# theartful/polychase

Measured on AMD Instinct MI355X. Metric: optical-flow frames/sec, higher is better.
Workload: dtype u8/int32 fixed-point + f32 2x2 solve; 1 GPU; C2 1920x1080 300-frame synthetic clip, 3-level pyramidal LK (max_level=3); width=1920, height=1080, max_level=3, window=10, pairs_per_frame=8, frames_per_gpu=1877, arith=opencv_x86, parallelism=single GPU

## Files before the change

### polychase_amd/csrc/hip/api.hip

```cpp
#include "api_internal.hpp"

#include <dirent.h>
#include <unistd.h>

#include <cstring>
#include <mutex>

namespace pc {
std::string& last_error() {
    thread_local std::string e;
    return e;
}
}

namespace pc_api {

int collect_timing(pc_context* c) {
    if (c->ranges.empty()) return PC_OK;
    PC_HIP(c->sync_side_streams());
    PC_HIP(hipStreamSynchronize(c->stream));
    std::vector<std::pair<float, float>> spans[PC_K_COUNT];
    hipEvent_t const origin = c->ranges.front().a;
    for (auto& r : c->ranges) {
        float ms = 0.f, t0 = 0.f;
// ... 105 lines not shown

static bool tiled_response(const pc_gftt_options& opt) {
    static const bool force_general = getenv("POLYCHASE_GFTT_GENERAL") && atoi(getenv("POLYCHASE_GFTT_GENERAL")) == 1;
    return opt.block_size == 3 && opt.gradient_size == 3 && !opt.use_harris && !force_general;
}

static bool fused_detection(const pc_gftt_options& opt) {
    return tiled_response(opt) && opt.min_distance >= 1 && !(opt.min_distance > pc::kSuppressMaxTableRadius);
}

static int corner_response(pc_context* ctx, const pc_frame* f, DetectScratch& d, const pc::GfttGrid& grid, const pc_gftt_options& opt,
                           uint32_t* cell_max) {
    const int fma = ((ctx->arith & PC_ARITH_SOBEL_FMA) ? 1 : 0) | ((ctx->arith & PC_ARITH_SOBEL_ROW_FMA) ? 2 : 0);
    if (tiled_response(opt)) {
        pc::launch_min_eig(f->levels[0], d.eig.p, grid, cell_max, fma, ctx->work);
        return PC_OK;
    }
    PC_HIP(d.cov.ensure((size_t)3 * f->w * f->h));
    const bool two_pass = opt.block_size >= pc::kBoxRowsFromBlock;
    if (two_pass) PC_HIP(d.box_rows.ensure((size_t)3 * f->w * f->h));
    if (!pc::launch_corner_response(f->levels[0], d.eig.p, d.cov.p, two_pass ? d.box_rows.p : nullptr, grid, cell_max, opt.block_size, opt.gradient_size, opt.use_harris != 0, opt.harris_k,
                                    fma, ctx->work))
        return fail(PC_E_INVALID, "gradient_size must be 3, 5, 7 (Sobel) or -1 (Scharr)");
    return PC_OK;
}

int detect_reserve(pc_context* ctx, int w, int h, DetectScratch& d, const pc_gftt_options* opt) {
    const size_t npx = (size_t)w * h;
    const size_t cand_cap = std::min(npx, npx / 4 + 65536);
    PC_HIP(d.eig.ensure(npx));
    PC_HIP(d.cstate.ensure(npx + 16));
    PC_HIP(d.keys.ensure(cand_cap));
    PC_HIP(d.keys_bucketed.ensure(cand_cap));
    if (opt && fused_detection(*opt)) PC_HIP(d.key_slots.ensure((size_t)pc::kSortBuckets * pc::kBucketSlots, true));
    PC_HIP(d.keys_sorted.ensure(cand_cap));
    d.cand_cap = (uint32_t)std::min<size_t>(d.keys.cap, std::min(d.keys_bucketed.cap, d.keys_sorted.cap));
    d.ticket_stride = ticket_stride(w, h, d.cand_cap);
    d.counter_words = kTicketsAt + 3 * (int)d.ticket_stride;
    PC_HIP(d.counters.ensure((size_t)d.counter_words));
    PC_HIP(d.bucket_offsets.ensure(pc::kSortBuckets + 1));
    PC_HIP(d.per_block.ensure((size_t)pc::suppress_num_blocks(d.cand_cap) + 1));
    PC_HIP(d.h_counters.ensure(kHostCells));
    if (!d.ev_b) PC_HIP(hipEventCreateWithFlags(&d.ev_b, hipEventDisableTiming));
    (void)ctx;
    return PC_OK;
}

static int upload_suppression_offsets(pc_context* ctx, const pc_gftt_options& opt) {
    if (!(opt.min_distance >= 1) || ctx->sup_min_distance == opt.min_distance) return PC_OK;
    if (opt.min_distance > pc::kSuppressMaxTableRadius) return PC_OK;
    const std::vector<int2> offs = suppression_offsets(opt.min_distance);
    PC_HIP(ctx->sup_offsets.ensure(offs.size() + 1));
    PC_HIP(hipStreamSynchronize(ctx->work));
    PC_HIP(hipMemcpy(ctx->sup_offsets.p, offs.data(), offs.size() * sizeof(int2), hipMemcpyHostToDevice));
    ctx->n_sup_offsets = (int)offs.size();
    int R = 0;
    for (const int2& o : offs) R = std::max(R, std::max(std::abs(o.x), std::abs(o.y)));
    std::vector<int> hw((size_t)2 * R + 1, -1);
    for (const int2& o : offs) hw[(size_t)(o.y + R)] = std::max(hw[(size_t)(o.y + R)], std::abs(o.x));
    hw[(size_t)R] = std::max(hw[(size_t)R], 0);
    size_t covered = 0;
    for (int v : hw) covered += v >= 0 ? (size_t)(2 * v + 1) : 0;
    if (covered != offs.size() + 1) return fail(PC_E_INVALID, "suppression neighbourhood is not row-contiguous");
    PC_HIP(ctx->sup_rows.ensure(hw.size()));
    PC_HIP(hipMemcpy(ctx->sup_rows.p, hw.data(), hw.size() * sizeof(int), hipMemcpyHostToDevice));
    ctx->sup_R = R;
    ctx->sup_min_distance = opt.min_distance;
    return PC_OK;
}

static int ensure_perm_capacity(pc_frame* f, int n) {
    if (f->perm_cap >= n) return PC_OK;
    if (f->d_perm) PC_HIP(hipFree(f->d_perm));
    f->d_perm = nullptr;
    f->perm_cap = 0;
    const int want = std::max(n + n / 2, 1024);
    PC_HIP(hipMalloc(&f->d_perm, (size_t)want * 2 * sizeof(uint32_t)));
    f->perm_cap = want;
    return PC_OK;
}

int detect_enqueue(pc_context* ctx, pc_frame* f, const pc::GfttGrid& grid, const pc_gftt_options& opt, DetectScratch& d,
                   DevBuf<uint32_t>& hist, bool full_launch) {
    const int w = f->w, h = f->h;
    int rc = detect_reserve(ctx, w, h, d, &opt);
    if (rc != PC_OK) return rc;
    if ((rc = upload_suppression_offsets(ctx, opt)) != PC_OK) return rc;
    if (f->kp_cap < 4096 && (rc = ensure_kp_capacity(f, 4096)) != PC_OK) return rc;
    if ((rc = ensure_perm_capacity(f, f->kp_cap)) != PC_OK) return rc;
    PC_HIP(hist.ensure((size_t)pc::bin_num_tiles(w, h) + 1));
    uint32_t* const cnt = d.counters.p;
    if (!d.cleared) PC_HIP(hipMemsetAsync(cnt, 0, (size_t)d.counter_words * sizeof(uint32_t), ctx->work));
    uint32_t* const tickets = cnt + kTicketsAt;
    d.cleared = false;
    const uint32_t n_launch = (ctx->cand_hint > 0 && !full_launch) ? std::min(ctx->cand_hint, d.cand_cap) : d.cand_cap;
    const bool large_radius = opt.min_distance > pc::kSuppressMaxTableRadius;
    const bool fused = fused_detection(opt);
    {
        ScopedTimer t(ctx, PC_K_MINEIG);
        if ((rc = corner_response(ctx, f, d, grid, opt, cnt + kCellMaxAt)) != PC_OK) return rc;
    }
    {
        ScopedTimer t(ctx, PC_K_NMS);
        pc::launch_nms(d.eig.p, w, h, grid, cnt + kCellMaxAt, opt.quality_level, d.keys.p, d.cand_cap, cnt + kCntCand, d.cstate.p,
                       cnt + kCntSortParams, cnt + kHistAt, tickets, d.bucket_offsets.p, hist.p, ctx->work,
                       fused ? d.key_slots.p : nullptr, fused ? d.per_block.p : nullptr, pc::suppress_num_blocks(n_launch));
    }
    {
        ScopedTimer t(ctx, PC_K_SORT);
        if (fused)
            pc::launch_bucket_sort_slots(d.key_slots.p, d.bucket_offsets.p, d.keys_sorted.p, cnt + kCntOverflow, ctx->work);
        else
            pc::launch_bucket_sort(d.keys.p, d.cand_cap, n_launch, cnt + kCntCand, cnt + kCntSortParams, d.bucket_offsets.p,
                                   cnt + kCursorAt, d.keys_bucketed.p, d.keys_sorted.p, cnt + kCntOverflow, ctx->work);
    }
    const uint32_t limit = opt.max_corners > 0 ? std::min<uint32_t>((uint32_t)opt.max_corners, (uint32_t)f->kp_cap) : (uint32_t)f->kp_cap;
    if (large_radius) PC_HIP(d.sup_grid.ensure((size_t)pc::suppress_large_grid_words(w, h, opt.min_distance)));
    if (fused) {
        ScopedTimer t(ctx, PC_K_SUPPRESS);
        pc::launch_suppress_compact(d.keys_sorted.p, n_launch, cnt + kCntCand, w, h, d.eig.p, d.cstate.p, ctx->sup_offsets.p,
                                    ctx->n_sup_offsets, ctx->sup_rows.p, ctx->sup_R, d.per_block.p, cnt + kCntStuck, limit, f->d_kps,
                                    cnt + kCntKps, hist.p, cnt + kCntOverflow, tickets + d.ticket_stride, ctx->work);
    } else {
        ScopedTimer t(ctx, PC_K_SUPPRESS);
        pc::launch_suppress_and_compact(d.keys_sorted.p, n_launch, cnt + kCntCand, w, h, d.eig.p, d.cstate.p, ctx->sup_offsets.p,
                                        ctx->n_sup_offsets, ctx->sup_rows.p, ctx->sup_R, opt.min_distance >= 1, d.per_block.p,
                                        cnt + kCntStuck, limit, f->d_kps,
                                        cnt + kCntKps, hist.p, cnt + kCntOverflow, tickets + d.ticket_stride, d.ticket_stride,
                                        opt.min_distance, large_radius ? d.sup_grid.p : nullptr, ctx->work);
    }
    pc::launch_spatial_bins_counted(f->d_kps, (int)std::min<uint32_t>(limit, n_launch), cnt + kCntKps, w, h, hist.p, f->d_perm,
                                    f->d_perm + f->perm_cap, cnt, d.h_counters.p, kHostCells, ctx->work);
    PC_HIP(hipEventRecord(d.ev_b, ctx->work));
    f->n_kps = -1;
    f->n_cands = -1;
    f->perm_valid = false;
    return PC_OK;
}

static int detect_slow_path(pc_context* ctx, pc_frame* f, const pc::GfttGrid& grid, const pc_gftt_options& opt, DetectScratch& d,
                            DevBuf<uint32_t>& hist) {
    const int w = f->w, h = f->h;
    const uint32_t npx = (uint32_t)((size_t)w * h);
    PC_HIP(hipStreamSynchronize(ctx->work));
    PC_HIP(d.keys.ensure(npx));
    PC_HIP(d.keys_sorted.ensure(npx));
    PC_HIP(d.per_block.ensure((size_t)pc::suppress_num_blocks(npx) + 1));
    PC_HIP(hist.ensure((size_t)pc::bin_num_tiles(w, h) + 1));
    uint32_t* const cnt = d.counters.p;
    d.cleared = false;
    PC_HIP(hipMemsetAsync(cnt, 0, (size_t)d.counter_words * sizeof(uint32_t), ctx->work));
    uint32_t* const tickets = cnt + kTicketsAt;
    if (int crc = corner_response(ctx, f, d, grid, opt, cnt + kCellMaxAt)) return crc;
// ... 831 lines not shown
```

### polychase_amd/csrc/hip/kernels.hpp

```cpp
#pragma once

#include "bvh.hpp"
#include "common.hpp"

namespace pc {

int helper_prio_arg();
void set_helper_prio(int hi);

void launch_rgb2gray(const uint8_t* rgb, size_t rgb_pitch, const Level& l0, hipStream_t s);
void launch_rgbf32_to_gray(const float* rgb, size_t rgb_pitch, int channels, const Level& l0, hipStream_t s);
void launch_copy_gray(const uint8_t* gray, size_t gray_pitch, const Level& l0, hipStream_t s);
void launch_pyrdown(const Level& src, const Level& dst, hipStream_t s);
void launch_border(const Level& l, int win, hipStream_t s);
void launch_widen(const Level& l, int win, hipStream_t s);
void launch_scharr(const Level& l, hipStream_t s);

enum LevelSourceKind { SRC_PYR = 0, SRC_RGB8 = 1, SRC_GRAY8 = 2, SRC_RGBF32 = 3 };
struct LevelSource {
    int kind;
    const uint8_t* src;
    size_t src_pitch;
    int channels;
    int aligned;
    Level parent;
    uint32_t* clear;
    int clear_words;
};
void launch_level(const LevelSource& in, const Level& out, int win, hipStream_t s);

struct GfttGrid {
    int rows, cols;
    int cell_w, cell_h;
};
constexpr int kMaxGridCells = 1024;
void launch_min_eig(const Level& l0, float* eig, const GfttGrid& g, uint32_t* cell_max, int sobel_fma, hipStream_t s);
constexpr int kBoxRowsFromBlock = 12;
bool launch_corner_response(const Level& l0, float* eig, float* cov, double* box_rows, const GfttGrid& g, uint32_t* cell_max, int block_size, int gradient_size,
                            bool harris, double harris_k, int sobel_fma, hipStream_t s);
constexpr int kSortBuckets = 8192;
constexpr int kBucketSlots = 512;
void launch_nms(const float* eig, int w, int h, const GfttGrid& g, const uint32_t* cell_max, double quality_level,
                unsigned long long* keys, uint32_t cap, uint32_t* counter, uint8_t* cstate, uint32_t* sort_params, uint32_t* hist,
                uint32_t* ticket, uint32_t* bucket_offsets, uint32_t* bin_hist, hipStream_t s,
                unsigned long long* slots = nullptr, uint32_t* zero = nullptr, int zero_words = 0);
void launch_bucket_sort(const unsigned long long* keys, uint32_t cap, uint32_t n_launch, const uint32_t* counter, const uint32_t* sort_params,
                        const uint32_t* offsets, uint32_t* cursor, unsigned long long* scratch, unsigned long long* out,
                        uint32_t* overflow, hipStream_t s);
void launch_bucket_sort_slots(const unsigned long long* slots, const uint32_t* offsets, unsigned long long* out, uint32_t* overflow,
                              hipStream_t s);
int suppress_num_blocks(uint32_t n);
void launch_suppress_and_compact(const unsigned long long* keys, uint32_t n_max, const uint32_t* n_dev, int w, int h, const float* eig,
                                 uint8_t* cstate, const int2* offsets, int n_offsets, const int* row_hw, int R, bool suppress,
                                 uint32_t* per_block,
                                 uint32_t* stuck, uint32_t max_corners, float2* xy, uint32_t* n_out, uint32_t* bin_hist,
                                 uint32_t* overflow, uint32_t* tickets, uint32_t ticket_stride, double large_min_distance, uint32_t* large_grid,
                                 hipStream_t s);
void launch_suppress_compact(const unsigned long long* keys, uint32_t n_max, const uint32_t* n_dev, int w, int h, const float* eig,
                             uint8_t* cstate, const int2* offsets, int n_offsets, const int* row_hw, int R, uint32_t* lookback,
                             uint32_t* stuck, uint32_t max_corners, float2* xy, uint32_t* n_out, uint32_t* bin_hist,
                             uint32_t* overflow, uint32_t* ticket, hipStream_t s);
constexpr double kSuppressMaxTableRadius = 64.0;
int suppress_large_grid_words(int w, int h, double min_distance);
hipError_t sort_keys_desc(void* temp, size_t& temp_bytes, unsigned long long* keys_in,
                          unsigned long long* keys_out, uint32_t n, hipStream_t s);

constexpr int kMaxLevels = 16;
struct LKParams {
    Level src[kMaxLevels];
    const uint8_t* tgt[8][kMaxLevels];
    const uint16_t* tgt16[8][kMaxLevels];
    int n_targets;
    int max_level;
    int n;
    const float2* pts;
    const uint32_t* perm;
    int blocks_per_xcd;
    int max_iters;
    double eps_sq;
    float min_eig_thr;
    float min_eig_num_thr;
    float4* out_rec;
    unsigned long long* prof;
    uint32_t* gate;
    uint32_t gate_value;
    int x86_order;
    unsigned long long* x86_stats;
};
void launch_lk_gate(const uint32_t* gate, uint32_t value, uint32_t* timed_out, hipStream_t s);
__device__ __forceinline__ void lk_signal_dispatched(const LKParams& p) {
    if (p.gate && blockIdx.x == gridDim.x - 1 && threadIdx.x == 0)
        __hip_atomic_store(p.gate, p.gate_value, __ATOMIC_RELAXED, __HIP_MEMORY_SCOPE_AGENT);
// ... 135 lines not shown
```

### polychase_amd/csrc/hip/kernels_gftt.hip

```cpp
#include <algorithm>
#include <cstring>
#include <type_traits>
#include <rocprim/device/device_radix_sort.hpp>

#include <cmath>

#include "kernels.hpp"

namespace pc {

constexpr int TW = 64, TH = 16;
constexpr int GH = TH + 4, G_PITCH = 72;
constexpr int CW = TW + 2, CH = TH + 2;

template <bool ROW_FMA>
__device__ __forceinline__ float smooth_row(float a, float b, float c, float f1, float f0) {
    float t = f1 * a;
    if (ROW_FMA) {
        t = __fmaf_rn(f0, b, t);
        t = __fmaf_rn(f1, c, t);
    } else {
        t += f0 * b;
        t += f1 * c;
    }
// ... 496 lines not shown
    if (box_rows) hipLaunchKernelGGL(box_rows_kernel, grid, dim3(256), 0, s, cov, l0.w, l0.h, block_size, box_rows, helper_prio_arg());
    hipLaunchKernelGGL(box_response_kernel, grid, dim3(256), 0, s, cov, (const double*)box_rows, l0.w, l0.h, block_size, harris ? ((sobel_fma & 1) ? 2 : 1) : 0, harris_k, eig, g, cell_max,
                       helper_prio_arg());
    return true;
}

constexpr int NMS_SUB = 4;

struct SortRange {
    uint32_t hi, shift;
};
__host__ __device__ __forceinline__ SortRange make_sort_range(uint32_t lo, uint32_t hi) {
    SortRange r;
    r.hi = hi;
    r.shift = 0;
    const uint32_t span = hi > lo ? hi - lo : 0u;
    while ((span >> r.shift) >= (uint32_t)kSortBuckets) r.shift++;
    return r;
}
__device__ __forceinline__ uint32_t bucket_of(uint32_t ord, const SortRange& r) {
    const uint32_t d = r.hi > ord ? r.hi - ord : 0u;
    const uint32_t b = d >> r.shift;
    return b < (uint32_t)kSortBuckets ? b : (uint32_t)kSortBuckets - 1u;
}

__global__ __launch_bounds__(256) void nms_kernel(const float* __restrict__ eig, int w, int h, GfttGrid g,
                                                  const uint32_t* __restrict__ cell_max, double quality_level,
                                                  unsigned long long* __restrict__ keys, uint32_t cap,
                                                  uint32_t* __restrict__ counter, uint8_t* __restrict__ cstate,
                                                  uint32_t* __restrict__ sort_params, uint32_t* __restrict__ hist,
                                                  uint32_t* __restrict__ ticket, uint32_t* __restrict__ bucket_offsets,
                                                  uint32_t* __restrict__ bin_hist, int n_tiles,
                                                  unsigned long long* __restrict__ slots, uint32_t* __restrict__ zero, int zero_words,
                                                  int hi_prio) {
    helper_priority(hi_prio);
    __shared__ float s_thr[kMaxGridCells];
    __shared__ uint32_t s_hi, s_lo;
    __shared__ float s_v[CH][CW + 2];
    __shared__ uint32_t s_wave[4];
    __shared__ uint32_t s_base;
    const int tid = threadIdx.x;
    const int x0 = blockIdx.x * TW;
    const int ncells = g.rows * g.cols;
    if (tid == 0) {
        s_hi = 0u;
        s_lo = 0xffffffffu;
    }
    __syncthreads();
    for (int i = tid; i < ncells; i += 256) {
        const float mx = ordered_to_float(cell_max[i]);
        s_thr[i] = (float)((double)mx * quality_level);
        atomicMax(&s_hi, cell_max[i]);
        atomicMin(&s_lo, float_to_ordered(s_thr[i] > 0.f ? s_thr[i] : 0.f));
    }
    __syncthreads();
    const SortRange range = make_sort_range(s_lo, s_hi);
    if (blockIdx.x == 0 && blockIdx.y == 0) {
        if (tid == 0) {
            sort_params[0] = range.hi;
            sort_params[1] = range.shift;
        }
        if (bin_hist)
            for (int i = tid; i < n_tiles; i += 256) bin_hist[i] = 0u;
    }
    for (int i = (blockIdx.y * gridDim.x + blockIdx.x) * 256 + tid; i < zero_words; i += gridDim.x * gridDim.y * 256) zero[i] = 0u;
    const int r = tid >> 4, q = tid & 15;
    const int x = x0 + 4 * q;
// ... 93 lines not shown
        s_base = total ? atomicAdd(counter, total) : 0u;
    }
    __syncthreads();
    if (cnt != 0) {
        uint32_t pos = s_base + incl - cnt;
        for (int wv = 0; wv < wave; wv++) pos += s_wave[wv];
#pragma unroll
        for (int sub = 0; sub < NMS_SUB; sub++) {
            const int y = (blockIdx.y * NMS_SUB + sub) * TH + r;
#pragma unroll
            for (int i = 0; i < 4; i++) {
                if (flags & (1u << (4 * sub + i))) {
                    const uint32_t ord = float_to_ordered(vals[sub][i]);
                    if (pos < cap) {
                        const unsigned long long key = ((unsigned long long)ord << 32) | (unsigned long long)(uint32_t)(y * w + x + i);
                        const uint32_t b = bucket_of(ord, range);
                        if (slots) {
                            const uint32_t at = atomicAdd(&hist[b], 1u);
                            slots[(size_t)b * kBucketSlots + min(at, (uint32_t)kBucketSlots - 1u)] = key;
                        } else {
                            keys[pos] = key;
                            atomicAdd(&hist[b], 1u);
                        }
                    }
                    pos++;
                }
            }
        }
    }
    if (ticket && last_workgroup(ticket, gridDim.x * gridDim.y)) {
        __shared__ uint32_t s_scan[256];
        const uint32_t total = scan_exclusive_256_fixed<kSortBuckets / 256>(hist, bucket_offsets, s_scan);
        if (tid == 0) bucket_offsets[kSortBuckets] = total;
    }
}

void launch_nms(const float* eig, int w, int h, const GfttGrid& g, const uint32_t* cell_max, double quality_level,
                unsigned long long* keys, uint32_t cap, uint32_t* counter, uint8_t* cstate, uint32_t* sort_params, uint32_t* hist,
                uint32_t* ticket, uint32_t* bucket_offsets, uint32_t* bin_hist, hipStream_t s,
                unsigned long long* slots, uint32_t* zero, int zero_words) {
    dim3 grid((w + TW - 1) / TW, (h + NMS_SUB * TH - 1) / (NMS_SUB * TH));
    hipLaunchKernelGGL(nms_kernel, grid, dim3(256), 0, s, eig, w, h, g, cell_max, quality_level, keys, cap, counter, cstate,
                       sort_params, hist, ticket, bucket_offsets, bin_hist, bin_hist ? bin_num_tiles(w, h) : 0, slots, zero,
                       zero ? zero_words : 0, helper_prio_arg());
}

constexpr int kBucketLds = 512;

__global__ __launch_bounds__(256) void bucket_scatter_kernel(const unsigned long long* __restrict__ keys, uint32_t cap,
                                                             const uint32_t* __restrict__ counter, const uint32_t* __restrict__ sort_params,
                                                             const uint32_t* __restrict__ offsets, uint32_t* __restrict__ cursor,
                                                             unsigned long long* __restrict__ out, int hi_prio) {
    helper_priority(hi_prio);
    const uint32_t n = min(*counter, cap);
    SortRange range;
    range.hi = sort_params[0];
    range.shift = sort_params[1];
    for (uint32_t i = blockIdx.x * blockDim.x + threadIdx.x; i < n; i += gridDim.x * blockDim.x) {
        const unsigned long long key = keys[i];
        const uint32_t b = bucket_of((uint32_t)(key >> 32), range);
        out[offsets[b] + atomicAdd(&cursor[b], 1u)] = key;
    }
}

constexpr int kBucketsPerWave = 4;

constexpr int kSortWaves = 4;
static_assert(kBucketSlots == kBucketLds, "a bucket beyond its slots is a bucket beyond the fast path");
template <bool SLOTS>
__global__ __launch_bounds__(64 * kSortWaves) void bucket_sort_kernel(const unsigned long long* __restrict__ in, const uint32_t* __restrict__ offsets,
                                                         unsigned long long* __restrict__ out, uint32_t* __restrict__ overflow, int hi_prio) {
    helper_priority(hi_prio);
    __shared__ unsigned long long s_all[kSortWaves][kBucketLds];
    const int lane = threadIdx.x & 63, wave = threadIdx.x >> 6;
    unsigned long long* const s_keys = s_all[wave];
    const int b0 = (blockIdx.x * kSortWaves + wave) * kBucketsPerWave;
    if (b0 >= kSortBuckets) return;
// ... 73 lines not shown
                        uint32_t* overflow, hipStream_t s) {
    const unsigned blocks = std::max(1u, std::min<unsigned>(1024u, (n_launch + 255u) / 256u));
    hipLaunchKernelGGL(bucket_scatter_kernel, dim3(blocks), dim3(256), 0, s, keys, cap, counter, sort_params, offsets, cursor, scratch, helper_prio_arg());
    hipLaunchKernelGGL(bucket_sort_kernel<false>, dim3((kSortBuckets / kBucketsPerWave + kSortWaves - 1) / kSortWaves), dim3(64 * kSortWaves), 0, s, scratch,
                       offsets, out, overflow, helper_prio_arg());
}
void launch_bucket_sort_slots(const unsigned long long* slots, const uint32_t* offsets, unsigned long long* out, uint32_t* overflow,
                              hipStream_t s) {
    hipLaunchKernelGGL(bucket_sort_kernel<true>, dim3((kSortBuckets / kBucketsPerWave + kSortWaves - 1) / kSortWaves), dim3(64 * kSortWaves), 0, s, slots,
                       offsets, out, overflow, helper_prio_arg());
}

struct AcceptedScan {
    uint32_t* ticket;
    uint32_t* n_out;
    uint32_t* overflow;
    uint32_t max_corners;
};
__device__ __forceinline__ void finish_accepted_scan(uint32_t* per_block, const AcceptedScan& fin, uint32_t n_max, const uint32_t* n_dev) {
    if (!last_workgroup(fin.ticket, gridDim.x)) return;
    __shared__ uint32_t s_scan[256];
    if (threadIdx.x == 0 && n_dev && fin.overflow && *n_dev > n_max) atomicOr(fin.overflow, 4u);
    const uint32_t total = scan_exclusive_256(per_block, per_block, (int)gridDim.x, s_scan);
    if (threadIdx.x == 0) *fin.n_out = (fin.max_corners > 0 && total > fin.max_corners) ? fin.max_corners : total;
}

constexpr uint8_t CS_CAND = 1, CS_ACCEPTED = 2, CS_REJECTED = 3;
constexpr int SUP_NB = 12;
constexpr int SUP_BLOCK = 256;

__device__ __forceinline__ uint8_t cs_load(const uint8_t* p) { return __hip_atomic_load(p, __ATOMIC_RELAXED, __HIP_MEMORY_SCOPE_AGENT); }
__device__ __forceinline__ void cs_store(uint8_t* p, uint8_t v) { __hip_atomic_store(p, v, __ATOMIC_RELAXED, __HIP_MEMORY_SCOPE_AGENT); }

__device__ __forceinline__ bool suppress_decide(const unsigned long long* __restrict__ keys, uint32_t n, int w, int h,
                                                const float* __restrict__ eig, uint8_t* cstate, const int2* __restrict__ offsets,
                                                int n_offsets, const int* __restrict__ row_hw, int R, uint32_t* __restrict__ stuck,
                                                uint32_t* idx_out) {
    const uint32_t i = blockIdx.x * SUP_BLOCK + threadIdx.x;
    const bool live = i < n;
    uint32_t my_val = 0, my_idx = 0;
    uint32_t nb[SUP_NB];
    int n_nb = 0;
    bool overflow = false;
    int x = 0, y = 0;
    if (live) {
        const unsigned long long key = keys[i];
        my_val = (uint32_t)(key >> 32);
        my_idx = (uint32_t)key;
        y = (int)(my_idx / (uint32_t)w);
        x = (int)(my_idx - (uint32_t)y * (uint32_t)w);
        for (int dy = -R; dy <= R; dy++) {
            const int ny = y + dy, hw = row_hw[dy + R];
            if (ny < 0 || ny >= h || hw < 0) continue;
            const uint32_t lin0 = (uint32_t)(ny * w + max(x - hw, 0)), lin1 = (uint32_t)(ny * w + min(x + hw, w - 1));
            for (uint32_t a = lin0 & ~3u; a <= lin1; a += 4u) {
                uint32_t v = *reinterpret_cast<const uint32_t*>(cstate + a);
                if (a < lin0) v &= 0xffffffffu << (8u * (lin0 - a));
                if (a + 3u > lin1) v &= 0xffffffffu >> (8u * (a + 3u - lin1));
                while (v) {
                    const uint32_t b = (uint32_t)(__ffs((int)v) - 1) >> 3;
                    v &= ~(0xffu << (8u * b));
                    const uint32_t nidx = a + b;
                    if (nidx == my_idx) continue;
                    const uint32_t nval = float_to_ordered(eig[nidx]);
                    if (!(nval > my_val || (nval == my_val && nidx > my_idx))) continue;
                    if (n_nb < SUP_NB) {
#pragma unroll
                        for (int k = 0; k < SUP_NB; k++)
                            if (k == n_nb) nb[k] = nidx;
                        n_nb++;
                    } else {
                        overflow = true;
                    }
                }
            }
        }
    }
    bool done = !live;
    bool accepted = false;
// ... 19 lines not shown
                        const uint8_t st = cs_load(&cstate[nb[k]]);
                        rejected |= (st == CS_ACCEPTED);
                        blocked |= (st == CS_CAND);
                    }
                }
            }
            if (rejected || !blocked) {
                cs_store(&cstate[my_idx], rejected ? CS_REJECTED : CS_ACCEPTED);
                accepted = !rejected;
                done = true;
            }
        }
        if (__all(done)) break;
        if (spin > (1u << 22)) {
            if (!done) atomicAdd(stuck, 1u);
            break;
        }
        __builtin_amdgcn_s_sleep(1);
    }
    *idx_out = my_idx;
    return accepted;
}

__global__ __launch_bounds__(SUP_BLOCK) void suppress_sorted_kernel(const unsigned long long* __restrict__ keys, uint32_t n_max,
                                                                    const uint32_t* __restrict__ n_dev, int w, int h,
                                                                    const float* __restrict__ eig, uint8_t* cstate,
                                                                    const int2* __restrict__ offsets, int n_offsets,
                                                                    const int* __restrict__ row_hw, int R,
                                                                    uint32_t* __restrict__ accepted_per_block,
                                                                    uint32_t* __restrict__ stuck, AcceptedScan fin, int hi_prio) {
    helper_priority(hi_prio);
    const uint32_t n = n_dev ? min(*n_dev, n_max) : n_max;
    uint32_t idx;
    const bool accepted = suppress_decide(keys, n, w, h, eig, cstate, offsets, n_offsets, row_hw, R, stuck, &idx);
    const int c = __syncthreads_count(accepted);
    if (threadIdx.x == 0) publish(&accepted_per_block[blockIdx.x], (uint32_t)c);
    finish_accepted_scan(accepted_per_block, fin, n_max, n_dev);
}

constexpr uint32_t kLbAggregate = 1u << 30, kLbPrefix = 1u << 31, kLbCount = kLbAggregate - 1u;
__device__ __forceinline__ uint32_t lookback_exclusive(uint32_t* lookback, uint32_t b, uint32_t c, uint32_t* __restrict__ stuck) {
    const int lane = (int)(threadIdx.x & 63);
    if (b == 0) {
        if (lane == 0) publish(&lookback[0], kLbPrefix | c);
        return 0u;
    }
    if (lane == 0) publish(&lookback[b], kLbAggregate | c);
    uint32_t excl = 0;
    int top = (int)b - 1;
    for (uint32_t spin = 0;; spin++) {
        const int j = top - lane;
        const uint32_t v = j >= 0 ? __hip_atomic_load(&lookback[j], __ATOMIC_RELAXED, __HIP_MEMORY_SCOPE_AGENT) : kLbPrefix;
        const unsigned long long pre = __ballot((v & kLbPrefix) != 0u);
        const int stop = pre ? __ffsll((long long)pre) - 1 : 63;
        const unsigned long long upto = stop == 63 ? ~0ull : ((2ull << stop) - 1ull);
        if ((__ballot(v == 0u) & upto) == 0ull) {
            uint32_t part = lane <= stop ? (v & kLbCount) : 0u;
#pragma unroll
            for (int d = 32; d >= 1; d >>= 1) part += __shfl_xor(part, d);
            excl += part;
            if (pre) break;
            top -= 64;
            continue;
        }
        if (spin > (1u << 22)) {
            if (lane == 0) atomicAdd(stuck, 1u);
            break;
        }
        __builtin_amdgcn_s_sleep(1);
    }
    if (lane == 0) publish(&lookback[b], kLbPrefix | (excl + c));
    return excl;
}

__global__ __launch_bounds__(SUP_BLOCK) void suppress_compact_kernel(const unsigned long long* __restrict__ keys, uint32_t n_max,
                                                                     const uint32_t* __restrict__ n_dev, int w, int h,
                                                                     const float* __restrict__ eig, uint8_t* cstate,
                                                                     const int2* __restrict__ offsets, int n_offsets,
                                                                     const int* __restrict__ row_hw, int R, uint32_t* lookback,
                                                                     uint32_t* __restrict__ stuck, uint32_t max_corners,
                                                                     float2* __restrict__ xy, uint32_t* __restrict__ n_out,
                                                                     uint32_t* __restrict__ bin_hist, int tiles_x, int n_tiles,
                                                                     uint32_t* __restrict__ overflow, uint32_t* __restrict__ ticket,
                                                                     int hi_prio) {
    helper_priority(hi_prio);
    __shared__ uint32_t s_wave[SUP_BLOCK / 64];
    __shared__ uint32_t s_excl;
    const uint32_t n_all = n_dev ? *n_dev : n_max;
    const bool redo = (overflow && (*overflow & 1u) != 0u) || n_all > n_max;
    const uint32_t n = redo ? 0u : n_all;
    if (blockIdx.x * SUP_BLOCK < n) {
        uint32_t idx;
        const bool accepted = suppress_decide(keys, n, w, h, eig, cstate, offsets, n_offsets, row_hw, R, stuck, &idx);
        const unsigned long long ballot = __ballot(accepted);
        const int lane = threadIdx.x & 63, wave = threadIdx.x >> 6;
        if (lane == 0) s_wave[wave] = (uint32_t)__popcll(ballot);
        __syncthreads();
        if (wave == 0) {
            uint32_t c = 0;
#pragma unroll
            for (int wv = 0; wv < SUP_BLOCK / 64; wv++) c += s_wave[wv];
            const uint32_t excl = lookback_exclusive(lookback, blockIdx.x, c, stuck);
            if (lane == 0) s_excl = excl;
        }
        __syncthreads();
        if (accepted) {
            uint32_t pos = s_excl + (uint32_t)__popcll(ballot & ((1ull << lane) - 1ull));
            for (int wv = 0; wv < wave; wv++) pos += s_wave[wv];
            if (!(max_corners > 0 && pos >= max_corners)) {
                const uint32_t y = idx / (uint32_t)w, x = idx - y * (uint32_t)w;
                xy[pos] = make_float2((float)x, (float)y);
                if (bin_hist) atomicAdd(&bin_hist[min(n_tiles - 1, (int)((y >> 6) * tiles_x + (x >> 6)))], 1u);
            }
        }
    }
    if (last_workgroup(ticket, gridDim.x)) {
        __shared__ uint32_t s_scan[256];
        if (threadIdx.x == 0) {
            const uint32_t total =
                n ? (__hip_atomic_load(&lookback[(n - 1u) / SUP_BLOCK], __ATOMIC_RELAXED, __HIP_MEMORY_SCOPE_AGENT) & kLbCount) : 0u;
            *n_out = (max_corners > 0 && total > max_corners) ? max_corners : total;
            if (n_dev && overflow && *n_dev > n_max) atomicOr(overflow, 4u);
        }
        if (bin_hist) (void)scan_exclusive_256(bin_hist, bin_hist, n_tiles, s_scan);
    }
}
// ... 129 lines not shown
}
int suppress_large_grid_words(int w, int h, double min_distance) {
    const int cell = suppress_large_cell(w, h, min_distance);
    return ((w + cell - 1) / cell) * ((h + cell - 1) / cell) * kLargeCellWords;
}

int suppress_num_blocks(uint32_t n) { return (int)((n + SUP_BLOCK - 1) / SUP_BLOCK); }

void launch_suppress_and_compact(const unsigned long long* keys, uint32_t n_max, const uint32_t* n_dev, int w, int h, const float* eig,
                                 uint8_t* cstate, const int2* offsets, int n_offsets, const int* row_hw, int R, bool suppress,
                                 uint32_t* per_block,
                                 uint32_t* stuck, uint32_t max_corners, float2* xy, uint32_t* n_out, uint32_t* bin_hist,
                                 uint32_t* overflow, uint32_t* tickets, uint32_t ticket_stride, double large_min_distance, uint32_t* large_grid,
                                 hipStream_t s) {
    uint32_t* const accepted_per_block = per_block;
    const int nb = suppress_num_blocks(n_max);
    if (nb == 0) return;
    const AcceptedScan fin{tickets, n_out, overflow, max_corners};
    if (suppress && large_grid) {
        const int cell = suppress_large_cell(w, h, large_min_distance), gw = (w + cell - 1) / cell, gh = (h + cell - 1) / cell;
        (void)hipMemsetAsync(large_grid, 0, (size_t)gw * gh * kLargeCellWords * sizeof(uint32_t), s);
        hipLaunchKernelGGL(suppress_large_radius_kernel, dim3(1), dim3(256), 0, s, keys, n_max, n_dev, w, cstate, large_min_distance * large_min_distance,
                           cell, gw, gh, large_grid, accepted_per_block, nb, stuck, n_out, overflow, max_corners, helper_prio_arg());
    } else if (suppress)
        hipLaunchKernelGGL(suppress_sorted_kernel, dim3(nb), dim3(SUP_BLOCK), 0, s, keys, n_max, n_dev, w, h, eig, cstate, offsets,
                           n_offsets, row_hw, R, accepted_per_block, stuck, fin, helper_prio_arg());
    else
        hipLaunchKernelGGL(accept_all_kernel, dim3(nb), dim3(SUP_BLOCK), 0, s, keys, n_max, n_dev, cstate, accepted_per_block, fin, helper_prio_arg());
    const int tiles_x = (w + 63) >> 6, n_tiles = bin_hist ? bin_num_tiles(w, h) : 0;
    hipLaunchKernelGGL(accepted_scatter_kernel, dim3(nb), dim3(SUP_BLOCK), 0, s, keys, n_max, n_dev, w, cstate, per_block, max_corners, xy,
                       bin_hist, tiles_x, n_tiles, tickets + ticket_stride, helper_prio_arg());
}

void launch_suppress_compact(const unsigned long long* keys, uint32_t n_max, const uint32_t* n_dev, int w, int h, const float* eig,
                             uint8_t* cstate, const int2* offsets, int n_offsets, const int* row_hw, int R, uint32_t* lookback,
                             uint32_t* stuck, uint32_t max_corners, float2* xy, uint32_t* n_out, uint32_t* bin_hist,
                             uint32_t* overflow, uint32_t* ticket, hipStream_t s) {
    const int nb = suppress_num_blocks(n_max);
    if (nb == 0) return;
    const int tiles_x = (w + 63) >> 6, n_tiles = bin_hist ? bin_num_tiles(w, h) : 0;
    hipLaunchKernelGGL(suppress_compact_kernel, dim3(nb), dim3(SUP_BLOCK), 0, s, keys, n_max, n_dev, w, h, eig, cstate, offsets, n_offsets,
                       row_hw, R, lookback, stuck, max_corners, xy, n_out, bin_hist, tiles_x, n_tiles, overflow, ticket, helper_prio_arg());
}

hipError_t sort_keys_desc(void* temp, size_t& temp_bytes, unsigned long long* keys_in,
                          unsigned long long* keys_out, uint32_t n, hipStream_t s) {
    return rocprim::radix_sort_keys_desc(temp, temp_bytes, keys_in, keys_out, (size_t)n, 0u, 64u, s);
}

}
```

Baseline: 3431 frames/s.

## Fuse per-bucket slot sort into suppression kernel, dropping separate sort pass

Removes the separate bucket-sort-slots kernel on the fused detection path. Each suppression block now finds the buckets covering its sorted output positions using coarse and fine offset tables written by the NMS scan, loads those slots into LDS and ranks them within each bucket. The slot-overflow check moves into the NMS kernel. This saves a kernel launch and a global round trip for the sorted keys, at the cost of extra LDS use, redundant loads of bucket tails shared by neighbouring blocks, and more complex lookup logic in the suppression kernel.

```diff
diff --git a/polychase_amd/csrc/hip/api.hip b/polychase_amd/csrc/hip/api.hip
--- a/polychase_amd/csrc/hip/api.hip
+++ b/polychase_amd/csrc/hip/api.hip
@@ -161,13 +161,14 @@
     PC_HIP(d.cstate.ensure(npx + 16));
     PC_HIP(d.keys.ensure(cand_cap));
     PC_HIP(d.keys_bucketed.ensure(cand_cap));
-    if (opt && fused_detection(*opt)) PC_HIP(d.key_slots.ensure((size_t)pc::kSortBuckets * pc::kBucketSlots, true));
-    PC_HIP(d.keys_sorted.ensure(cand_cap));
-    d.cand_cap = (uint32_t)std::min<size_t>(d.keys.cap, std::min(d.keys_bucketed.cap, d.keys_sorted.cap));
+    const bool fused = opt && fused_detection(*opt);
+    if (fused) PC_HIP(d.key_slots.ensure((size_t)pc::kSortBuckets * pc::kBucketSlots, true));
+    if (!fused) PC_HIP(d.keys_sorted.ensure(cand_cap));
+    d.cand_cap = (uint32_t)std::min<size_t>(d.keys.cap, fused ? d.keys_bucketed.cap : std::min(d.keys_bucketed.cap, d.keys_sorted.cap));
     d.ticket_stride = ticket_stride(w, h, d.cand_cap);
     d.counter_words = kTicketsAt + 3 * (int)d.ticket_stride;
     PC_HIP(d.counters.ensure((size_t)d.counter_words));
-    PC_HIP(d.bucket_offsets.ensure(pc::kSortBuckets + 1));
+    PC_HIP(d.bucket_offsets.ensure(pc::kSortOffsetWords));
     PC_HIP(d.per_block.ensure((size_t)pc::suppress_num_blocks(d.cand_cap) + 1));
     PC_HIP(d.h_counters.ensure(kHostCells));
     if (!d.ev_b) PC_HIP(hipEventCreateWithFlags(&d.ev_b, hipEventDisableTiming));
@@ -233,21 +234,19 @@
         ScopedTimer t(ctx, PC_K_NMS);
         pc::launch_nms(d.eig.p, w, h, grid, cnt + kCellMaxAt, opt.quality_level, d.keys.p, d.cand_cap, cnt + kCntCand, d.cstate.p,
                        cnt + kCntSortParams, cnt + kHistAt, tickets, d.bucket_offsets.p, hist.p, ctx->work,
-                       fused ? d.key_slots.p : nullptr, fused ? d.per_block.p : nullptr, pc::suppress_num_blocks(n_launch));
-    }
-    {
+                       fused ? d.key_slots.p : nullptr, fused ? d.per_block.p : nullptr, pc::suppress_num_blocks(n_launch),
+                       cnt + kCntOverflow);
+    }
+    if (!fused) {
         ScopedTimer t(ctx, PC_K_SORT);
-        if (fused)
-            pc::launch_bucket_sort_slots(d.key_slots.p, d.bucket_offsets.p, d.keys_sorted.p, cnt + kCntOverflow, ctx->work);
-        else
-            pc::launch_bucket_sort(d.keys.p, d.cand_cap, n_launch, cnt + kCntCand, cnt + kCntSortParams, d.bucket_offsets.p,
-                                   cnt + kCursorAt, d.keys_bucketed.p, d.keys_sorted.p, cnt + kCntOverflow, ctx->work);
+        pc::launch_bucket_sort(d.keys.p, d.cand_cap, n_launch, cnt + kCntCand, cnt + kCntSortParams, d.bucket_offsets.p,
+                               cnt + kCursorAt, d.keys_bucketed.p, d.keys_sorted.p, cnt + kCntOverflow, ctx->work);
     }
     const uint32_t limit = opt.max_corners > 0 ? std::min<uint32_t>((uint32_t)opt.max_corners, (uint32_t)f->kp_cap) : (uint32_t)f->kp_cap;
     if (large_radius) PC_HIP(d.sup_grid.ensure((size_t)pc::suppress_large_grid_words(w, h, opt.min_distance)));
     if (fused) {
         ScopedTimer t(ctx, PC_K_SUPPRESS);
-        pc::launch_suppress_compact(d.keys_sorted.p, n_launch, cnt + kCntCand, w, h, d.eig.p, d.cstate.p, ctx->sup_offsets.p,
+        pc::launch_suppress_compact(d.key_slots.p, d.bucket_offsets.p, n_launch, cnt + kCntCand, w, h, d.eig.p, d.cstate.p, ctx->sup_offsets.p,
                                     ctx->n_sup_offsets, ctx->sup_rows.p, ctx->sup_R, d.per_block.p, cnt + kCntStuck, limit, f->d_kps,
                                     cnt + kCntKps, hist.p, cnt + kCntOverflow, tickets + d.ticket_stride, ctx->work);
     } else {
diff --git a/polychase_amd/csrc/hip/kernels.hpp b/polychase_amd/csrc/hip/kernels.hpp
--- a/polychase_amd/csrc/hip/kernels.hpp
+++ b/polychase_amd/csrc/hip/kernels.hpp
@@ -40,10 +40,12 @@
                             bool harris, double harris_k, int sobel_fma, hipStream_t s);
 constexpr int kSortBuckets = 8192;
 constexpr int kBucketSlots = 512;
+constexpr int kSortCoarse = 32;
+constexpr int kSortOffsetWords = kSortBuckets + 1 + kSortBuckets / kSortCoarse;
 void launch_nms(const float* eig, int w, int h, const GfttGrid& g, const uint32_t* cell_max, double quality_level,
                 unsigned long long* keys, uint32_t cap, uint32_t* counter, uint8_t* cstate, uint32_t* sort_params, uint32_t* hist,
                 uint32_t* ticket, uint32_t* bucket_offsets, uint32_t* bin_hist, hipStream_t s,
-                unsigned long long* slots = nullptr, uint32_t* zero = nullptr, int zero_words = 0);
+                unsigned long long* slots = nullptr, uint32_t* zero = nullptr, int zero_words = 0, uint32_t* overflow = nullptr);
 void launch_bucket_sort(const unsigned long long* keys, uint32_t cap, uint32_t n_launch, const uint32_t* counter, const uint32_t* sort_params,
                         const uint32_t* offsets, uint32_t* cursor, unsigned long long* scratch, unsigned long long* out,
                         uint32_t* overflow, hipStream_t s);
@@ -56,8 +58,8 @@
                                  uint32_t* stuck, uint32_t max_corners, float2* xy, uint32_t* n_out, uint32_t* bin_hist,
                                  uint32_t* overflow, uint32_t* tickets, uint32_t ticket_stride, double large_min_distance, uint32_t* large_grid,
                                  hipStream_t s);
-void launch_suppress_compact(const unsigned long long* keys, uint32_t n_max, const uint32_t* n_dev, int w, int h, const float* eig,
-                             uint8_t* cstate, const int2* offsets, int n_offsets, const int* row_hw, int R, uint32_t* lookback,
+void launch_suppress_compact(const unsigned long long* slots, const uint32_t* bucket_offsets, uint32_t n_max, const uint32_t* n_dev, int w, int h,
+                             const float* eig, uint8_t* cstate, const int2* offsets, int n_offsets, const int* row_hw, int R, uint32_t* lookback,
                              uint32_t* stuck, uint32_t max_corners, float2* xy, uint32_t* n_out, uint32_t* bin_hist,
                              uint32_t* overflow, uint32_t* ticket, hipStream_t s);
 constexpr double kSuppressMaxTableRadius = 64.0;
diff --git a/polychase_amd/csrc/hip/kernels_gftt.hip b/polychase_amd/csrc/hip/kernels_gftt.hip
--- a/polychase_amd/csrc/hip/kernels_gftt.hip
+++ b/polychase_amd/csrc/hip/kernels_gftt.hip
@@ -552,7 +552,7 @@
                                                   uint32_t* __restrict__ ticket, uint32_t* __restrict__ bucket_offsets,
                                                   uint32_t* __restrict__ bin_hist, int n_tiles,
                                                   unsigned long long* __restrict__ slots, uint32_t* __restrict__ zero, int zero_words,
-                                                  int hi_prio) {
+                                                  uint32_t* __restrict__ overflow, int hi_prio) {
     helper_priority(hi_prio);
     __shared__ float s_thr[kMaxGridCells];
     __shared__ uint32_t s_hi, s_lo;
@@ -712,17 +712,28 @@
         __shared__ uint32_t s_scan[256];
         const uint32_t total = scan_exclusive_256_fixed<kSortBuckets / 256>(hist, bucket_offsets, s_scan);
         if (tid == 0) bucket_offsets[kSortBuckets] = total;
+        static_assert(kSortBuckets / 256 == kSortCoarse, "one coarse offset per lane of the scan");
+        bucket_offsets[kSortBuckets + 1 + tid] = bucket_offsets[tid * kSortCoarse];
+        if (slots && overflow) {
+            bool beyond = false;
+#pragma unroll
+            for (int k = 0; k < kSortBuckets / 256 / 4; k++) {
+                const uint4 c = reinterpret_cast<const uint4*>(hist + tid * (kSortBuckets / 256))[k];
+                beyond |= max(max(c.x, c.y), max(c.z, c.w)) > (uint32_t)kBucketSlots;
+            }
+            if (__any(beyond) && (tid & 63) == 0) atomicOr(overflow, 1u);
+        }
     }
 }
 
 void launch_nms(const float* eig, int w, int h, const GfttGrid& g, const uint32_t* cell_max, double quality_level,
                 unsigned long long* keys, uint32_t cap, uint32_t* counter, uint8_t* cstate, uint32_t* sort_params, uint32_t* hist,
                 uint32_t* ticket, uint32_t* bucket_offsets, uint32_t* bin_hist, hipStream_t s,
-                unsigned long long* slots, uint32_t* zero, int zero_words) {
+                unsigned long long* slots, uint32_t* zero, int zero_words, uint32_t* overflow) {
     dim3 grid((w + TW - 1) / TW, (h + NMS_SUB * TH - 1) / (NMS_SUB * TH));
     hipLaunchKernelGGL(nms_kernel, grid, dim3(256), 0, s, eig, w, h, g, cell_max, quality_level, keys, cap, counter, cstate,
                        sort_params, hist, ticket, bucket_offsets, bin_hist, bin_hist ? bin_num_tiles(w, h) : 0, slots, zero,
-                       zero ? zero_words : 0, helper_prio_arg());
+                       zero ? zero_words : 0, overflow, helper_prio_arg());
 }
 
 constexpr int kBucketLds = 512;
@@ -862,19 +873,16 @@
 __device__ __forceinline__ uint8_t cs_load(const uint8_t* p) { return __hip_atomic_load(p, __ATOMIC_RELAXED, __HIP_MEMORY_SCOPE_AGENT); }
 __device__ __forceinline__ void cs_store(uint8_t* p, uint8_t v) { __hip_atomic_store(p, v, __ATOMIC_RELAXED, __HIP_MEMORY_SCOPE_AGENT); }
 
-__device__ __forceinline__ bool suppress_decide(const unsigned long long* __restrict__ keys, uint32_t n, int w, int h,
+__device__ __forceinline__ bool suppress_decide(bool live, unsigned long long key, int w, int h,
                                                 const float* __restrict__ eig, uint8_t* cstate, const int2* __restrict__ offsets,
                                                 int n_offsets, const int* __restrict__ row_hw, int R, uint32_t* __restrict__ stuck,
                                                 uint32_t* idx_out) {
-    const uint32_t i = blockIdx.x * SUP_BLOCK + threadIdx.x;
-    const bool live = i < n;
     uint32_t my_val = 0, my_idx = 0;
     uint32_t nb[SUP_NB];
     int n_nb = 0;
     bool overflow = false;
     int x = 0, y = 0;
     if (live) {
-        const unsigned long long key = keys[i];
         my_val = (uint32_t)(key >> 32);
         my_idx = (uint32_t)key;
         y = (int)(my_idx / (uint32_t)w);
@@ -960,7 +968,8 @@
     helper_priority(hi_prio);
     const uint32_t n = n_dev ? min(*n_dev, n_max) : n_max;
     uint32_t idx;
-    const bool accepted = suppress_decide(keys, n, w, h, eig, cstate, offsets, n_offsets, row_hw, R, stuck, &idx);
+    const uint32_t i = blockIdx.x * SUP_BLOCK + threadIdx.x;
+    const bool accepted = suppress_decide(i < n, i < n ? keys[i] : 0ull, w, h, eig, cstate, offsets, n_offsets, row_hw, R, stuck, &idx);
     const int c = __syncthreads_count(accepted);
     if (threadIdx.x == 0) publish(&accepted_per_block[blockIdx.x], (uint32_t)c);
     finish_accepted_scan(accepted_per_block, fin, n_max, n_dev);
@@ -1001,7 +1010,108 @@
     return excl;
 }
 
-__global__ __launch_bounds__(SUP_BLOCK) void suppress_compact_kernel(const unsigned long long* __restrict__ keys, uint32_t n_max,
+constexpr int kSupLoadMax = SUP_BLOCK + 2 * (kBucketSlots - 1);
+constexpr int kSupLoadPerLane = (kSupLoadMax + SUP_BLOCK - 1) / SUP_BLOCK;
+struct SupSortLds {
+    unsigned long long in[kSupLoadPerLane * SUP_BLOCK];
+    unsigned long long sorted[SUP_BLOCK];
+    uint32_t start[SUP_BLOCK + 1];
+    uint32_t bucket[SUP_BLOCK];
+    uint32_t wave_cnt[2][SUP_BLOCK / 64];
+};
+__device__ __forceinline__ void suppress_sort_front(const unsigned long long* __restrict__ slots, const uint32_t* __restrict__ offs,
+                                                    uint32_t n, SupSortLds& L) {
+    const int tid = threadIdx.x, lane = tid & 63, wave = tid >> 6;
+    const uint32_t p0 = blockIdx.x * SUP_BLOCK, p_last = min(p0 + SUP_BLOCK, n) - 1u;
+    constexpr int kFine = kSortCoarse, kCoarse = kSortBuckets / kFine;
+    static_assert(kCoarse % 64 == 0 && kFine * 2 == 64, "whole probe rounds, then half a wavefront per position");
+    uint32_t c0 = 0, c1 = 0;
+    uint32_t probe[kCoarse / 64];
+#pragma unroll
+    for (int q = 0; q < kCoarse / 64; q++) probe[q] = offs[kSortBuckets + 1 + lane + 64 * q];
+#pragma unroll
+    for (int q = 0; q < kCoarse / 64; q++) {
+        c0 += (uint32_t)__popcll(__ballot(probe[q] <= p0));
+        c1 += (uint32_t)__popcll(__ballot(probe[q] <= p_last));
+    }
+    const uint32_t fine = offs[kFine * ((lane < kFine ? c0 : c1) - 1u) + (lane & (kFine - 1))];
+    const unsigned long long le = __ballot(fine <= (lane < kFine ? p0 : p_last));
+    const uint32_t b_first = kFine * (c0 - 1u) + (uint32_t)__popcll(le & 0xffffffffull) - 1u;
+    const uint32_t b_last = kFine * (c1 - 1u) + (uint32_t)__popcll(le >> 32) - 1u;
+    const uint32_t base = __shfl(fine, (int)(b_first & (kFine - 1)));
+    uint32_t nb = 0;
+    for (uint32_t bb = b_first, it = 0; bb <= b_last; bb += SUP_BLOCK, it++) {
+        const uint32_t b = bb + tid;
+        uint32_t o = 0, o1 = 0;
+        if (b <= b_last) {
+            o = offs[b];
+            o1 = offs[b + 1u];
+        }
+        const unsigned long long some = __ballot(o1 > o);
+        if (lane == 0) L.wave_cnt[it & 1][wave] = (uint32_t)__popcll(some);
+        __syncthreads();
+        uint32_t k = nb + (uint32_t)__popcll(some & ((1ull << lane) - 1ull));
+#pragma unroll
+        for (int wv = 0; wv < SUP_BLOCK / 64; wv++) {
+            const uint32_t c = L.wave_cnt[it & 1][wv];
+            k += wv < wave ? c : 0u;
+            nb += c;
+        }
+        if (o1 > o && k < (uint32_t)SUP_BLOCK) {
+            L.start[k] = o - base;
+            L.bucket[k] = b;
+        }
+    }
+    nb = min(nb, (uint32_t)SUP_BLOCK);
+    const uint32_t m = min(offs[b_last + 1u] - base, (uint32_t)(kSupLoadPerLane * SUP_BLOCK));
+    if (tid == 0) L.start[nb] = m;
+    __syncthreads();
+    uint32_t steps = 0;
+    while ((1u << steps) < nb) steps++;
+    uint32_t kk[kSupLoadPerLane];
+    unsigned long long ld[kSupLoadPerLane];
+#pragma unroll
+    for (int q = 0; q < kSupLoadPerLane; q++) {
+        const uint32_t i = tid + SUP_BLOCK * q;
+        uint32_t lo = 0;
+        for (uint32_t st = steps; st-- > 0u;) {
+            const uint32_t mid = lo + (1u << st);
+            if (mid < nb && L.start[mid] <= i) lo = mid;
+        }
+        kk[q] = lo;
+        ld[q] = 0ull;
+        if (i < m) ld[q] = slots[(size_t)L.bucket[lo] * kBucketSlots + min(i - L.start[lo], (uint32_t)kBucketSlots - 1u)];
+    }
+#pragma unroll
+    for (int q = 0; q < kSupLoadPerLane; q++) {
+        const uint32_t i = tid + SUP_BLOCK * q;
+        if (i < m) L.in[i] = ld[q];
+    }
+    __syncthreads();
+#pragma unroll
+    for (int q = 0; q < kSupLoadPerLane; q++) {
+        const uint32_t i = tid + SUP_BLOCK * q;
+        if (__builtin_amdgcn_readfirstlane(i) >= m) break;
+        const bool have = i < m;
+        const uint32_t first = L.start[kk[q]], len = have ? L.start[kk[q] + 1u] - first : 1u;
+        uint32_t longest = have ? len : 0u;
+#pragma unroll
+        for (int d = 32; d >= 1; d >>= 1) longest = max(longest, (uint32_t)__shfl_xor((int)longest, d));
+        const unsigned long long mine = ld[q];
+        uint32_t rank = 0;
+#pragma unroll 8
+        for (uint32_t j = 0; j < longest; j++) {
+            const unsigned long long other = L.in[first + min(j, len - 1u)];
+            rank += (j < len && other > mine) ? 1u : 0u;
+        }
+        const uint32_t at = base + first + rank - p0;
+        if (have && at < (uint32_t)SUP_BLOCK) L.sorted[at] = mine;
+    }
+    __syncthreads();
+}
+
+__global__ __launch_bounds__(SUP_BLOCK) void suppress_compact_kernel(const unsigned long long* __restrict__ slots,
+                                                                     const uint32_t* __restrict__ bucket_offsets, uint32_t n_max,
                                                                      const uint32_t* __restrict__ n_dev, int w, int h,
                                                                      const float* __restrict__ eig, uint8_t* cstate,
                                                                      const int2* __restrict__ offsets, int n_offsets,
@@ -1014,12 +1124,15 @@
     helper_priority(hi_prio);
     __shared__ uint32_t s_wave[SUP_BLOCK / 64];
     __shared__ uint32_t s_excl;
+    __shared__ SupSortLds s_sort;
     const uint32_t n_all = n_dev ? *n_dev : n_max;
     const bool redo = (overflow && (*overflow & 1u) != 0u) || n_all > n_max;
     const uint32_t n = redo ? 0u : n_all;
     if (blockIdx.x * SUP_BLOCK < n) {
+        suppress_sort_front(slots, bucket_offsets, n, s_sort);
+        const bool live = blockIdx.x * SUP_BLOCK + threadIdx.x < n;
         uint32_t idx;
-        const bool accepted = suppress_decide(keys, n, w, h, eig, cstate, offsets, n_offsets, row_hw, R, stuck, &idx);
+        const bool accepted = suppress_decide(live, live ? s_sort.sorted[threadIdx.x] : 0ull, w, h, eig, cstate, offsets, n_offsets, row_hw, R, stuck, &idx);
         const unsigned long long ballot = __ballot(accepted);
         const int lane = threadIdx.x & 63, wave = threadIdx.x >> 6;
         if (lane == 0) s_wave[wave] = (uint32_t)__popcll(ballot);
@@ -1215,15 +1328,15 @@
                        bin_hist, tiles_x, n_tiles, tickets + ticket_stride, helper_prio_arg());
 }
 
-void launch_suppress_compact(const unsigned long long* keys, uint32_t n_max, const uint32_t* n_dev, int w, int h, const float* eig,
-                             uint8_t* cstate, const int2* offsets, int n_offsets, const int* row_hw, int R, uint32_t* lookback,
+void launch_suppress_compact(const unsigned long long* slots, const uint32_t* bucket_offsets, uint32_t n_max, const uint32_t* n_dev, int w, int h,
+                             const float* eig, uint8_t* cstate, const int2* offsets, int n_offsets, const int* row_hw, int R, uint32_t* lookback,
                              uint32_t* stuck, uint32_t max_corners, float2* xy, uint32_t* n_out, uint32_t* bin_hist,
                              uint32_t* overflow, uint32_t* ticket, hipStream_t s) {
     const int nb = suppress_num_blocks(n_max);
     if (nb == 0) return;
     const int tiles_x = (w + 63) >> 6, n_tiles = bin_hist ? bin_num_tiles(w, h) : 0;
-    hipLaunchKernelGGL(suppress_compact_kernel, dim3(nb), dim3(SUP_BLOCK), 0, s, keys, n_max, n_dev, w, h, eig, cstate, offsets, n_offsets,
-                       row_hw, R, lookback, stuck, max_corners, xy, n_out, bin_hist, tiles_x, n_tiles, overflow, ticket, helper_prio_arg());
+    hipLaunchKernelGGL(suppress_compact_kernel, dim3(nb), dim3(SUP_BLOCK), 0, s, slots, bucket_offsets, n_max, n_dev, w, h, eig, cstate, offsets,
+                       n_offsets, row_hw, R, lookback, stuck, max_corners, xy, n_out, bin_hist, tiles_x, n_tiles, overflow, ticket, helper_prio_arg());
 }
 
 hipError_t sort_keys_desc(void* temp, size_t& temp_bytes, unsigned long long* keys_in,
```

New measurement: 3253 frames/s. 5.2% lower.
